# ssilverman16/particle_col_image_segmentation

Measured on AMD Instinct MI355X. Metric: Mpixels/sec segmented (5-ch 1024x1024 TIFF), ROI mask IoU=1.0, higher is better.
Workload: dtype f32 planes / u8 class maps / int32 labels / f64 ROI sums; 1 GPU; BASELINE config 2: batch of 64 frames 1024x1024x5 float32 per GPU, full kernel chain, inputs resident in HBM; frames_per_gpu=64, height=1024, width=1024, planes=5, parallelism=frames x1, launch=one hipGraph replay per step, 4 in flight, tie_fallback_frames_last_step=0, reference_nan_frames_rank0=0

## Files before the change

include/pcseg.h:

```cpp
#ifndef PCSEG_H
#define PCSEG_H

#include <stddef.h>
#include <stdint.h>

#ifdef __cplusplus
extern "C" {
#endif

typedef void *pcseg_stream_t;

enum pcseg_status {
    PCSEG_OK = 0,
    PCSEG_ERR_ARG = -1,
    PCSEG_ERR_HIP = -2,
    PCSEG_ERR_WORKSPACE = -3,
    PCSEG_ERR_CAPACITY = -4
};

enum pcseg_region_col {
    PCSEG_R_AREA = 0, PCSEG_R_SUM_ROW = 1, PCSEG_R_SUM_COL = 2,
    PCSEG_R_MIN_ROW = 3, PCSEG_R_MIN_COL = 4, PCSEG_R_MAX_ROW1 = 5, PCSEG_R_MAX_COL1 = 6,
    PCSEG_R_FIRST = 7, PCSEG_R_NCOLS = 8
};
// ... 71 lines not shown
int pcseg_fill_holes(const uint8_t *mask, uint8_t *out, int B, int H, int W,
                     void *workspace, size_t workspace_bytes, pcseg_stream_t stream);

size_t pcseg_local_maxima_workspace_bytes(int B, int H, int W);
int pcseg_local_maxima_i32(const int32_t *img, uint8_t *is_max, int32_t *markers, int32_t *counts,
                           int B, int H, int W, void *workspace, size_t workspace_bytes, pcseg_stream_t stream);

enum pcseg_ws_poison { PCSEG_WS_POISON_BORDER = 8, PCSEG_WS_POISON_LABEL = 16, PCSEG_WS_POISON_LEVEL2 = 32 };
size_t pcseg_watershed_workspace_bytes(int B, int H, int W);
void pcseg_watershed_counters(int64_t *out, int reset);
int pcseg_watershed4_f32(const float *img, int64_t frame_stride, const int32_t *markers, const uint8_t *mask,
                         int32_t *out, int32_t *tie_flags, int B, int H, int W, int mode,
                         void *workspace, size_t workspace_bytes, pcseg_stream_t stream);

size_t pcseg_merge_groups_workspace_bytes(int B, int list_cap);
int pcseg_merge_groups(const int32_t *dilated_labels, int keys_are_roots, const int64_t *stats,
                       const int32_t *region_list, const int32_t *n_list, int32_t *group_of, int32_t *n_groups,
                       int B, int H, int W, int cap, int list_cap, void *workspace, size_t workspace_bytes,
                       pcseg_stream_t stream);
int pcseg_merge_groups_runs(const uint32_t *dilated_bits, const int32_t *run_parent, const int64_t *stats,
                            const int32_t *region_list, const int32_t *n_list, int32_t *group_of, int32_t *n_groups,
                            int B, int H, int W, int cap, int list_cap, void *workspace, size_t workspace_bytes,
                            pcseg_stream_t stream);

int pcseg_merge_groups_fused(const uint32_t *dilated_bits, const int32_t *run_parent, const int64_t *stats,
                             const int32_t *region_lists, const int32_t *n_lists, int slot, int n_slots,
                             int32_t *group_of, int32_t *n_groups, int64_t *group_stats, int B, int H, int W, int cap,
                             void *workspace, size_t workspace_bytes, pcseg_stream_t stream);

int pcseg_merge_groups_fused_multi(const uint32_t *dilated_bits, const int32_t *run_parent, const int64_t *stats,
                                   const int32_t *region_lists, const int32_t *n_lists, const int32_t *slots, int n_masks,
                                   int n_slots, int32_t *group_of, int32_t *n_groups, int64_t *group_stats, int B, int H,
                                   int W, int cap, void *workspace, size_t workspace_bytes, pcseg_stream_t stream);

int pcseg_group_reduce(const int64_t *stats, const int32_t *region_list, const int32_t *n_list,
                       const int32_t *group_of, const int32_t *n_groups, int64_t *group_stats,
                       int B, int H, int W, int cap, int list_cap, pcseg_stream_t stream);

int pcseg_classify_regions(const int64_t *stats, const uint8_t *cls_out, const int32_t *counts,
                           const uint8_t *class_slot, const uint8_t *class_particle,
                           const int32_t *min_cell, const int32_t *min_cluster, int n_slots,
                           uint8_t *kind, uint8_t *slot_of, int32_t *cells, int64_t *particle_area,
                           int64_t *type_stats, int32_t *region_list, int32_t *n_list, int32_t *nan_flag,
                           int B, int cap, pcseg_stream_t stream);

int pcseg_nearest_dist_f64(const double *a, int na, const double *b, int nb, double *out_a, pcseg_stream_t stream);

size_t pcseg_overlap_workspace_bytes(int B, int H, int W);
int pcseg_remove_overlapping(const uint8_t *dapi, const uint8_t *other, double threshold, uint8_t *out,
                             int B, int H, int W, void *workspace, size_t workspace_bytes,
                             pcseg_stream_t stream);

typedef struct pcseg_table_inputs {
    int32_t B, cap, C, n_ratios;
    const int64_t *frame_ids;
    const int32_t *counts; const int64_t *stats; const uint8_t *cls_out; const double *cc_sums;
    const uint8_t *kind; const uint8_t *slot_of; const int32_t *cells;
    const int64_t *particle_area; const int64_t *overlap_area; const int64_t *type_stats; const int32_t *tie_flags;
    const int32_t *region_list; const int32_t *n_list;
    const int32_t *group_of[5]; const int32_t *n_groups[5]; const int64_t *group_stats[5];
    const int32_t *n_markers; const int64_t *ws_stats; const double *ws_sums;
    int32_t ratio_num[8]; int32_t ratio_den[8][4];
    const int32_t *overflow; const int32_t *ws_overflow; const int32_t *nan_flag;
} pcseg_table_inputs;
size_t pcseg_table_workspace_bytes(int B, int cap);
int pcseg_table_layout(const pcseg_table_inputs *in, int64_t *totals, void *workspace, size_t workspace_bytes,
// ... 92 lines not shown
```

particle_col_image_segmentation_amd/_lib.py:

```python
import ctypes
import os
from ctypes import c_char_p, c_double, c_float, c_int, c_int64, c_size_t, c_uint64, c_void_p

_HERE = os.path.dirname(os.path.abspath(__file__))
LIB_PATH = os.path.join(_HERE, "libpcseg.so")
_lib = None


class PcsegError(RuntimeError):
    pass


_P = c_void_p
_I = c_int
SIGNATURES = {
    "pcseg_version": (c_int, []),
    "pcseg_last_error": (c_char_p, []),
    "pcseg_device_count": (c_int, []),
    "pcseg_timing_enable": (None, [c_int]),
    "pcseg_timing_report": (c_int, [c_char_p, c_size_t]),
    "pcseg_argmax_planes_f32": (c_int, [_P, _P, _I, _I, _I, _I, _P]),
    "pcseg_median5_u8": (c_int, [_P, _P, _I, _I, _I, _P]),
    "pcseg_classmap_label_workspace_bytes": (c_size_t, [_I, _I, _I]),
    "pcseg_classmap_label_f32": (c_int, [_P, _I, _P, _P, _P, _I, _I, _I, _P, c_size_t, _P]),
    "pcseg_ccl_workspace_bytes": (c_size_t, [_I, _I, _I]),
    "pcseg_ccl8_equal_u8": (c_int, [_P, _P, _P, _I, _I, _I, _P, c_size_t, _P]),
    "pcseg_ccl8_bool": (c_int, [_P, _P, _P, _I, _I, _I, _P, c_size_t, _P]),
    "pcseg_ccl4_bool": (c_int, [_P, _P, _P, _I, _I, _I, _P, c_size_t, _P]),
    "pcseg_compact_labels": (c_int, [_P, _P, _P, _I, _I, _I, _P, c_size_t, _P]),
    "pcseg_region_reduce": (c_int, [_P, _P, _P, _I, _I, _I, _I, _I, _P, _P, _P, _P, _P]),
    "pcseg_region_reduce_n": (c_int, [_P, _P, _P, _P, _I, _I, _I, _I, _I, _P, _P, _P, _P, _P]),
    "pcseg_region_reduce_sel": (c_int, [_P, _P, _P, ctypes.c_uint64, _P, _I, _I, _I, _I, _I, _P, _P, _P, _P, _P]),
    "pcseg_region_init": (c_int, [_P, _I, _I, _I, _I, _I, _P, _P, _P, _P]),
    "pcseg_region_sums2": (c_int, [_P, _P, ctypes.c_uint64, _I, _P, _P, _I, _P, _P, _P, _P, _I, _I, _I, _I, _P]),
    "pcseg_threshold_lt_f32": (c_int, [_P, c_float, _P, _I, _I, _I, _P]),
    "pcseg_edt_workspace_bytes": (c_size_t, [_I, _I, _I]),
    "pcseg_edt_sq_u8": (c_int, [_P, _P, _I, _I, _I, _I, _P, c_size_t, _P]),
    "pcseg_edt_sq_lt_f32": (c_int, [_P, c_int64, c_float, _P, _P, _I, _I, _I, _P, c_size_t, _P]),
    "pcseg_dilate_disk_u8": (c_int, [_P, c_uint64, _I, _P, _I, _I, _I, _P, c_size_t, _P]),
    "pcseg_fill_particle": (c_int, [_P, _P, _I, _I, _I, _I, _I, _P, _I, _I, _I, _P, c_size_t, _P]),
    "pcseg_fill_holes_workspace_bytes": (c_size_t, [_I, _I, _I]),
    "pcseg_fill_holes": (c_int, [_P, _P, _I, _I, _I, _P, c_size_t, _P]),
    "pcseg_local_maxima_workspace_bytes": (c_size_t, [_I, _I, _I]),
    "pcseg_local_maxima_i32": (c_int, [_P, _P, _P, _P, _I, _I, _I, _P, c_size_t, _P]),
    "pcseg_watershed_workspace_bytes": (c_size_t, [_I, _I, _I]),
    "pcseg_watershed_counters": (None, [_P, _I]),
    "pcseg_watershed4_f32": (c_int, [_P, c_int64, _P, _P, _P, _P, _I, _I, _I, _I, _P, c_size_t, _P]),
    "pcseg_merge_groups_workspace_bytes": (c_size_t, [_I, _I]),
    "pcseg_merge_groups": (c_int, [_P, _I, _P, _P, _P, _P, _P, _I, _I, _I, _I, _I, _P, c_size_t, _P]),
    "pcseg_dilate_ccl_workspace_bytes": (c_size_t, [_I, _I, _I]),
    "pcseg_dilate_ccl_roots_u8": (c_int, [_P, c_uint64, _I, _P, _I, _I, _I, _P, c_size_t, _P]),
    "pcseg_dilate_ccl_runs_workspace_bytes": (c_size_t, [_I, _I, _I]),
    "pcseg_dilate_ccl_runs_u8": (c_int, [_P, c_uint64, _I, _P, _P, _I, _I, _I, _P, c_size_t, _P]),
    "pcseg_merge_groups_runs": (c_int, [_P, _P, _P, _P, _P, _P, _P, _I, _I, _I, _I, _I, _P, c_size_t, _P]),
    "pcseg_dilate_ccl_runs_multi_u8": (c_int, [_P, _P, _I, _I, _P, _P, _I, _I, _I, _P, c_size_t, _P]),
    "pcseg_merge_groups_fused_multi": (c_int, [_P, _P, _P, _P, _P, _P, _I, _I, _P, _P, _P, _I, _I, _I, _I, _P, c_size_t, _P]),
    "pcseg_merge_groups_fused": (c_int, [_P, _P, _P, _P, _P, _I, _I, _P, _P, _P, _I, _I, _I, _I, _P, c_size_t, _P]),
    "pcseg_group_reduce": (c_int, [_P, _P, _P, _P, _P, _P, _I, _I, _I, _I, _I, _P]),
    "pcseg_classify_regions": (c_int, [_P, _P, _P, _P, _P, _P, _P, _I, _P, _P, _P, _P, _P, _P, _P, _P, _I, _I, _P]),
    "pcseg_nearest_dist_f64": (c_int, [_P, _I, _P, _I, _P, _P]),
    "pcseg_overlap_workspace_bytes": (c_size_t, [_I, _I, _I]),
    "pcseg_remove_overlapping": (c_int, [_P, _P, c_double, _P, _I, _I, _I, _P, c_size_t, _P]),
    "pcseg_table_workspace_bytes": (c_size_t, [_I, _I]),
    "pcseg_table_layout": (c_int, [_P, _P, _P, c_size_t, _P]),
    "pcseg_table_write": (c_int, [_P, _P, _P, _P, _P, _P, c_size_t, _P]),
    "pcseg_cell_distances": (c_int, [_P, c_int64, _I, _P, c_double, c_double, _P, _I, _P, c_size_t, _P]),
    "pcseg_neighbours_workspace_bytes": (c_size_t, [c_int64, _I, _I, _I]),
    "pcseg_point_neighbours": (c_int, [_P, _P, _P, _P, c_int64, _I, _I, c_double, _P, _I, _P, _P, _P, _P, c_size_t, _P]),
    "pcseg_neighbours_pack_cells": (c_int, [_P, _I, _P, _I, _P, c_size_t, _P, _P, _P, _P, _P]),
    "pcseg_label_parent_workspace_bytes": (c_size_t, [_I, _I, _I, _I]),
    "pcseg_label_parent": (c_int, [_P, _P, _P, _P, _P, _P, _P, _P, _P, _P, _P, _I, _I, _I, _I, _P, c_size_t, _P]),
    "pcseg_refined_workspace_bytes": (c_size_t, [_I, _I]),
    "pcseg_refined_layout": (c_int, [_P, _P, _P, c_size_t, _P]),
    "pcseg_refined_table_write": (c_int, [_P, _P, c_size_t, _P, _P, _P, _P, _P, _P, _P, _P, c_size_t, _P]),
    "pcseg_surface_workspace_bytes": (c_size_t, [_I, _I, _I]),
    "pcseg_surface_points": (c_int, [_P, c_uint64, _P, _P, _P, _P, _P, c_int64, _I, _I, _I, _P, c_size_t, _P]),
    "pcseg_surface_distances": (c_int, [_P, _P, _P, c_int64, _P, _P, _P, _I, _I, _I, c_double, _P, _I, _I, _P, _P, _P, _P, _P, _P,
                                        c_size_t, _P]),
    "pcseg_surface_thresholds": (c_int, [_P, _I, c_double, _P]),
    "pcseg_surface_shells_workspace_bytes": (c_size_t, [_I, _I, _I]),
    "pcseg_surface_shells": (c_int, [_P, _P, _P, _I, _I, _I, c_double, _P, _I, _P, _P, c_size_t, _P]),
    "pcseg_surface_pack_cells": (c_int, [_P, _I, _P, _I, _P, c_size_t, _P, _P, _P, _P, _P]),
    "pcseg_surface_pack_refined": (c_int, [_P, _I, _P, _P, c_int64, _I, _P, _P]),
    "pcseg_region_shape_workspace_bytes": (c_size_t, [_I, _I, _I]),
    "pcseg_region_shape": (c_int, [_P, _P, _P, _P, _I, _I, _I, _I, _P, c_size_t, _P]),
    "pcseg_shape_properties": (c_int, [_P, _P, _P, _P, _I, _I, _P]),
    "pcseg_region_hull_workspace_bytes": (c_size_t, [_I, _I, _I, _I]),
    "pcseg_region_hull": (c_int, [_P, _P, _P, _P, _P, _I, _I, _I, _I, _P, c_size_t, _P]),
    "pcseg_hull_properties": (c_int, [_P, _P, _P, _P, _I, _I, _P]),
    "pcseg_nearest_label_workspace_bytes": (c_size_t, [_I, _I, _I]),
    "pcseg_nearest_label_i32": (c_int, [_P, _P, _I, _P, _P, _P, _I, _I, _I, _P, c_size_t, _P]),
    "pcseg_territory_labels": (c_int, [_P, _P, c_int64, _P, c_int64, _P]),
    "pcseg_territory_reduce": (c_int, [_P, _P, _P, c_int64, _I, _P, _I, _I, _I, _P]),
    "pcseg_territory_pairs_workspace_bytes": (c_size_t, [_I, _I]),
    "pcseg_territory_pairs": (c_int, [_P, _P, c_int64, _I, _P, _P, _P, _I, _I, _I, _P, c_size_t, _P]),
    "pcseg_territory_pairs_write": (c_int, [_I, _P, _P, _I, _I, _P, _P, _P, _P, _I, _P, c_size_t, _P]),
    "pcseg_otsu_hist_f32":(c_int, [_P, _P, _P, _I, _I, _I, _P]),
    "pcseg_otsu_f32": (c_int, [_P, _P, _P, _P, _I, _I, _I, _P]),
    "pcseg_morph3x3": (c_int, [_P, _P, _I, _I, _I, _I, _P]),
}


class TableInputs(ctypes.Structure):
    _fields_ = [("B", ctypes.c_int32), ("cap", ctypes.c_int32), ("C", ctypes.c_int32), ("n_ratios", ctypes.c_int32),
                ("frame_ids", _P),
                ("counts", _P), ("stats", _P), ("cls_out", _P), ("cc_sums", _P),
                ("kind", _P), ("slot_of", _P), ("cells", _P),
                ("particle_area", _P), ("overlap_area", _P), ("type_stats", _P), ("tie_flags", _P),
                ("region_list", _P), ("n_list", _P),
                ("group_of", _P * 5), ("n_groups", _P * 5), ("group_stats", _P * 5),
                ("n_markers", _P), ("ws_stats", _P), ("ws_sums", _P),
                ("ratio_num", ctypes.c_int32 * 8), ("ratio_den", (ctypes.c_int32 * 4) * 8),
                ("overflow", _P), ("ws_overflow", _P), ("nan_flag", _P)]


class RefinedInputs(ctypes.Structure):
    _fields_ = [("B", ctypes.c_int32), ("cap", ctypes.c_int32), ("n_slots", ctypes.c_int32),
                ("frame_ids", _P),
                ("counts", _P), ("kind", _P), ("slot_of", _P), ("cells", _P),
                ("n_markers", _P), ("ws_stats", _P),
                ("parent", _P), ("parent_px", _P), ("n_overlap", _P), ("cls_r", _P),
                ("kind_r", _P), ("slot_r", _P), ("cells_r", _P), ("type_stats_r", _P),
                ("nan_flag_r", _P),
                ("parent_overflow", _P)]


def load():
    global _lib
    if _lib is not None:
        return _lib
    path = os.environ.get("PCSEG_LIB") or LIB_PATH
    if not os.path.exists(path):
        raise PcsegError(
            "libpcseg.so is not built (%s). Run `python -m particle_col_image_segmentation_amd.build` "
            "or __graft_entry__.build(); there is no CPU fallback." % path)
    lib = ctypes.CDLL(path)
    for name, (res, args) in SIGNATURES.items():
        fn = getattr(lib, name)
        fn.restype = res
        fn.argtypes = args
    _lib = lib
    return lib


def check(rc, what):
    if rc != 0:
        msg = load().pcseg_last_error()
        raise PcsegError("%s failed (%d): %s" % (what, rc, msg.decode() if msg else "?"))
```

particle_col_image_segmentation_amd/build.py:

```python
import os
import subprocess
import sys

HERE = os.path.dirname(os.path.abspath(__file__))
CSRC = os.path.join(HERE, "csrc")
SOURCES = ["stencil.hip", "ccl.hip", "reduce.hip", "edt.hip", "watershed.hip", "tables.hip", "frontend.hip", "neighbours.hip", "refined.hip", "surface.hip", "shape.hip", "hull.hip", "voronoi.hip"]
LIB = os.path.join(HERE, "libpcseg.so")


def _stale():
    if not os.path.exists(LIB):
        return True
    t = os.path.getmtime(LIB)
    deps = [os.path.join(CSRC, f) for f in SOURCES + ["common.h", "tile_ops.h", "table_common.h", "label_reduce.h"]]
    deps.append(os.path.join(HERE, "..", "include", "pcseg.h"))
    return any(os.path.getmtime(d) > t for d in deps)


def build(force=False, verbose=False, out_dir=None, extra_flags=None):
    lib_path = LIB if out_dir is None else os.path.join(out_dir, "libpcseg.so")
    if out_dir is None and not force and not _stale():
        return LIB
    hipcc = os.environ.get("HIPCC", "/opt/rocm/bin/hipcc")
    objs = []
    procs = []
    obj_dir = os.path.join(HERE, "build") if out_dir is None else os.path.join(out_dir, "build")
    os.makedirs(obj_dir, exist_ok=True)
    flags = (extra_flags if extra_flags is not None else os.environ.get("PCSEG_EXTRA_FLAGS", "")).split()
    for src in SOURCES:
        obj = os.path.join(obj_dir, src.replace(".hip", ".o"))
        cmd = [hipcc, "--offload-arch=gfx950", "-O3", "-fPIC", "-std=c++17"] + flags + [
            "-c", os.path.join(CSRC, src), "-o", obj]
        if verbose:
            print(" ".join(cmd), file=sys.stderr)
        procs.append((src, subprocess.Popen(cmd, stdout=subprocess.PIPE, stderr=subprocess.STDOUT)))
        objs.append(obj)
    for src, p in procs:
        out, _ = p.communicate()
        if p.returncode != 0:
            raise RuntimeError("hipcc failed on %s:\n%s" % (src, out.decode()))
    cmd = [hipcc, "--offload-arch=gfx950", "-shared", "-fPIC", "-o", lib_path] + objs
    subprocess.check_call(cmd)
    return lib_path


if __name__ == "__main__":
    print(build(force="--force" in sys.argv, verbose=True))
# ... 1 lines not shown
```

particle_col_image_segmentation_amd/csrc/ccl.hip:

```cpp
#include <type_traits>

#include "common.h"
#include "tile_ops.h"

namespace pcseg {

constexpr int SCAN_PIX = 1024;

struct KeyEqU8 {
    const uint8_t *p;
    int W;
    int64_t n;
    __device__ __forceinline__ int operator()(int b, int r, int c) const { return p[b * n + rowoff(r, W) + c]; }
};
struct KeyNzU8 {
    const uint8_t *p;
    int W;
    int64_t n;
    __device__ __forceinline__ int operator()(int b, int r, int c) const { return p[b * n + rowoff(r, W) + c] != 0; }
};
struct KeyZeroU8 {
    const uint8_t *p;
    int W;
    int64_t n;
// ... 487 lines not shown
    }
    plan->parent = ws.parent;
    plan->blockcount = ws.blockcount;
    plan->nblk = ws.nblk;
    plan->corrupt = ws.corrupt;
    return PCSEG_OK;
}

int ccl_equal_u8_finish(const uint8_t *in, const CclPlan &plan, bool tile_pass_done, int *labels, int *counts, int B, int H, int W,
                        hipStream_t s)
{
    const KeyEqU8 keyfn{in, W, (int64_t)H * W};
    PCSEG_CHECK_HIP(hipMemsetAsync(plan.corrupt, 0, sizeof(int) * (size_t)B, s));
    dim3 tgrid((W + CCL_TW - 1) / CCL_TW, (H + CCL_TH - 1) / CCL_TH, B);
    if (!tile_pass_done) {
        PCSEG_LAUNCH((ccl_tile_kernel<KeyEqU8, true>), tgrid, dim3(256), 0, s, keyfn, plan.parent, H, W);
        PCSEG_CHECK_LAUNCH();
    }
    if (tgrid.x > 1 || tgrid.y > 1) {
        const int64_t border_px = (int64_t)((H - 1) / CCL_TH) * W + (int64_t)2 * ((W - 1) / CCL_TW) * H;
        dim3 bgrid((unsigned)((border_px + 255) / 256), B);
        PCSEG_LAUNCH((ccl_border_kernel<KeyEqU8, true>), bgrid, dim3(256), 0, s, keyfn, plan.parent, H, W, plan.corrupt);
        PCSEG_CHECK_LAUNCH();
    }
    return ccl_compact(plan.parent, plan.blockcount, plan.nblk, labels, counts, PredAll(), true, B, H, W, s, plan.corrupt);
}

__global__ void __launch_bounds__(256) roots_to_parent_kernel(const int *__restrict__ roots, int *__restrict__ parent, int64_t total)
{
    int64_t i = (int64_t)blockIdx.x * blockDim.x + threadIdx.x;
    if (i < total) parent[i] = roots[i] - 1;
}

struct MaskSet {
    unsigned long long bits[4];
    int n;
};
template <bool VEC>
__global__ void __launch_bounds__(256) set_bits_kernel(const uint8_t *__restrict__ in, MaskSet masks, unsigned *__restrict__ bits,
                                                        int H, int W, int nch, int B)
{
    constexpr int COLS = VEC ? 4 : 1;
    const int c = (blockIdx.x * 256 + threadIdx.x) * COLS;
    const int ch = blockIdx.y, b = blockIdx.z;
    if (c >= W) return;
    const uint8_t *src = in + (int64_t)b * H * W + c;
    unsigned w[4][COLS];
#pragma unroll
    for (int m = 0; m < 4; ++m)
#pragma unroll
        for (int j = 0; j < COLS; ++j) w[m][j] = 0;
#pragma unroll 1
    for (int j0 = 0; j0 < 32; j0 += 8) {
        unsigned v8[8];
#pragma unroll
        for (int j = 0; j < 8; ++j) {
            const uint8_t *at = src + rowoff(min(ch * 32 + j0 + j, H - 1), W);
            v8[j] = VEC ? *reinterpret_cast<const unsigned *>(at) : (unsigned)*at;
        }
#pragma unroll
        for (int j = 0; j < 8; ++j) {
#pragma unroll
            for (int q = 0; q < COLS; ++q) {
                const unsigned a = (v8[j] >> (8 * q)) & 255u;
                const unsigned long long sel = a < 64 ? (1ull << a) : 0ull;
#pragma unroll
                for (int m = 0; m < 4; ++m)
                    if (m < masks.n && (masks.bits[m] & sel)) w[m][q] |= 1u << (j0 + j);
            }
        }
// ... 741 lines not shown
```

particle_col_image_segmentation_amd/csrc/common.h:

```cpp
#pragma once
#include <hip/hip_runtime.h>
#include <stdint.h>
#include <stdio.h>
#include <string.h>

#include "../../include/pcseg.h"

namespace pcseg {

constexpr int WAVE = 64;

void set_error(const char *fmt, ...);

#define PCSEG_CHECK_HIP(expr)                                                              \
    do {                                                                                   \
        hipError_t _e = (expr);                                                            \
        if (_e != hipSuccess) {                                                            \
            pcseg::set_error("%s failed: %s (%s:%d)", #expr, hipGetErrorString(_e), __FILE__, __LINE__); \
            return PCSEG_ERR_HIP;                                                          \
        }                                                                                  \
    } while (0)

#define PCSEG_CHECK_LAUNCH()                                                               \
    do {                                                                                   \
        hipError_t _e = hipGetLastError();                                                 \
        if (_e != hipSuccess) {                                                            \
            pcseg::set_error("kernel launch failed: %s (%s:%d)", hipGetErrorString(_e), __FILE__, __LINE__); \
            return PCSEG_ERR_HIP;                                                          \
        }                                                                                  \
    } while (0)

#define PCSEG_REQUIRE(cond, msg)                                                           \
    do {                                                                                   \
        if (!(cond)) {                                                                     \
            pcseg::set_error("%s: %s", __func__, msg);                                     \
            return PCSEG_ERR_ARG;                                                          \
        }                                                                                  \
    } while (0)

// ... 222 lines not shown
            a = ga;
        }
        if (pb != b) {
            if (gb != pb) __hip_atomic_store(par + b, gb, __ATOMIC_RELAXED, __HIP_MEMORY_SCOPE_AGENT);
            b = gb;
        }
    }
    walk_corrupt(corrupt);
    return false;
}
__device__ __forceinline__ void unite_glb(int *par, int a, int b, int *corrupt = nullptr)
{
    for (;;) {
        if (!find2_glb(par, a, b, corrupt)) return;
        if (a == b) return;
        if (a < b) { int t = a; a = b; b = t; }
        int old = atomicMin(par + a, b);
        if (old == a) return;
        if (!walk_ok(a, old)) { walk_corrupt(corrupt); return; }
        a = old;
    }
}

struct CclPlan {
    int *parent;
    int *blockcount;
    int nblk;
    int *corrupt;
};
int ccl_plan(void *workspace, size_t workspace_bytes, int B, int H, int W, CclPlan *plan, const char *who);
int ccl_equal_u8_finish(const uint8_t *in, const CclPlan &plan, bool tile_pass_done, int *labels, int *counts, int B, int H, int W,
                        hipStream_t s);

}
```

particle_col_image_segmentation_amd/csrc/reduce.hip:

```cpp
#include "label_reduce.h"

namespace pcseg {

constexpr int RED_MAXC = 8;
constexpr int RED_ROWS = 16;

__device__ __forceinline__ void atomic_min_i64(long long *p, long long v) { atomicMin(p, v); }
__device__ __forceinline__ void atomic_max_i64(long long *p, long long v) { atomicMax(p, v); }

__global__ void __launch_bounds__(256) region_init_kernel(long long *__restrict__ stats, double *__restrict__ sums,
                                                           const int *__restrict__ counts, int cap, int C, int H, int W)
{
    const int b = blockIdx.y;
    const int idx = blockIdx.x * blockDim.x + threadIdx.x;
    const int l = idx >> 3, f = idx & 7;
    int nl = counts ? min(counts[b], cap) : cap;
    if (l >= nl) return;
    stats[((int64_t)b * cap + l) * 8 + f] = f == 3 ? (long long)H : (f == 4 ? (long long)W : (f == 7 ? 0x7FFFFFFFFFFFFFFFLL : 0LL));
    if (sums && f < C) sums[((int64_t)b * cap + l) * C + f] = 0.0;
}

__global__ void __launch_bounds__(256) region_reduce_kernel(const int *__restrict__ labels, const float *__restrict__ planes,
                                                             const uint8_t *__restrict__ cls, unsigned long long sel, int C, int H,
                                                             int W, int cap, long long *__restrict__ stats,
// ... 554 lines not shown
}

constexpr int MG_THREADS = 1024, MG_LDS = 4096;

struct LabelKeys {
    const int *lab;
    __device__ __forceinline__ int key(int fb, long long y, long long x, int H, int W) const
    {
        return lab[(int64_t)fb * H * W + y * W + x];
    }
};
struct RootKeys {
    const int *parent;
    __device__ __forceinline__ int key(int fb, long long y, long long x, int H, int W) const
    {
        const int *par = parent + (int64_t)fb * H * W;
        int k = par[y * W + x];
        if (k >= 0) k = (unsigned)k < (unsigned)(H * W) ? walk_root(par, k) : -1;
        return k + 1;
    }
};
struct RunRoots {
    const unsigned *bits;
    const int *parent;
    __device__ __forceinline__ int key(int fb, long long y, long long x, int H, int W) const
    {
        const int nch = (H + 31) / 32;
        const unsigned word = bits[((int64_t)fb * nch + (int)(y >> 5)) * W + x];
        const int j = (int)(y & 31);
        if (!((word >> j) & 1u)) return 0;
        const unsigned below = ~word & ((1u << j) - 1u);
        const int start = below ? 32 - __clz(below) : 0;
        return walk_root(parent + (int64_t)fb * H * W, (int)((y - j + start) * W + x)) + 1;
    }
};

template <typename Source>
__device__ __forceinline__ int centroid_key(const Source &src, const long long *st, int r, int fb, int H, int W, int cap)
{
    if (r < 0 || r >= cap) return 0;
    const long long a = st[(int64_t)r * 8 + 0];
    if (a <= 0) return 0;
    const long long y = st[(int64_t)r * 8 + 1] / a, x = st[(int64_t)r * 8 + 2] / a;
    if (y < 0 || y >= H || x < 0 || x >= W) return 0;
    return src.key(fb, y, x, H, W);
}

__device__ __forceinline__ void group_row_clear(long long *t, int H, int W)
{
    t[0] = 0; t[1] = 0; t[2] = 0; t[3] = H; t[4] = W; t[5] = 0; t[6] = 0; t[7] = 0;
}
__device__ __forceinline__ void group_row_add(long long *t, const long long *s, int f)
{
    if (f < 3) atomicAdd((unsigned long long *)&t[f], (unsigned long long)s[f]);
    else if (f < 5) atomicMin(&t[f], s[f]);
    else if (f < 7) atomicMax(&t[f], s[f]);
    else atomicAdd((unsigned long long *)&t[f], 1ull);
}

struct GroupTables {
    int *key, *gid, *first;
};

template <int THREADS, bool SUMS>
__device__ __forceinline__ int group_by_key(const GroupTables &t, int R, int *gof, int *wsum, const int *lst, const long long *st,
                                            long long *gs, int H, int W)
// ... 390 lines not shown
                                                 group_of, n_groups, nullptr, B, H, W, cap, list_cap, workspace, workspace_bytes, stream);
}

int pcseg_merge_groups_runs(const uint32_t *dilated_bits, const int32_t *run_parent, const int64_t *stats,
                            const int32_t *region_list, const int32_t *n_list, int32_t *group_of, int32_t *n_groups, int B, int H,
                            int W, int cap, int list_cap, void *workspace, size_t workspace_bytes, pcseg_stream_t stream)
{
    PCSEG_REQUIRE(dilated_bits && run_parent && stats && region_list && n_list && group_of && n_groups && workspace && cap >= 1 &&
                      list_cap >= 1 && check_shape(B, H, W),
                  "bad arguments");
    return merge_groups_launch<RunRoots, false>("merge_groups_runs", RunRoots{dilated_bits, run_parent}, stats, region_list, n_list,
                                                MergeSlots{}, 1, 1, group_of, n_groups, nullptr, B, H, W, cap, list_cap, workspace,
                                                workspace_bytes, stream);
}

int pcseg_merge_groups_fused_multi(const uint32_t *dilated_bits, const int32_t *run_parent, const int64_t *stats,
                                   const int32_t *region_lists, const int32_t *n_lists, const int32_t *slots, int n_masks, int n_slots,
                                   int32_t *group_of, int32_t *n_groups, int64_t *group_stats, int B, int H, int W, int cap,
                                   void *workspace, size_t workspace_bytes, pcseg_stream_t stream)
{
    PCSEG_REQUIRE(dilated_bits && run_parent && stats && region_lists && n_lists && slots && group_of && n_groups && group_stats &&
                      workspace && cap >= 1 && n_slots >= 1 && n_masks >= 1 && n_masks <= 4 && check_shape(B, H, W),
                  "bad arguments (1..4 masks)");
    MergeSlots ms;
    for (int m = 0; m < 4; ++m) {
        ms.slot[m] = m < n_masks ? slots[m] : 0;
        PCSEG_REQUIRE(ms.slot[m] >= 0 && ms.slot[m] < n_slots, "list slot out of range");
    }
    return merge_groups_launch<RunRoots, true>("merge_groups_fused", RunRoots{dilated_bits, run_parent}, stats, region_lists, n_lists, ms,
                                               n_masks, n_slots, group_of, n_groups, group_stats, B, H, W, cap, cap, workspace,
                                               workspace_bytes, stream);
}

int pcseg_merge_groups_fused(const uint32_t *dilated_bits, const int32_t *run_parent, const int64_t *stats,
                             const int32_t *region_lists, const int32_t *n_lists, int slot, int n_slots, int32_t *group_of,
                             int32_t *n_groups, int64_t *group_stats, int B, int H, int W, int cap, void *workspace,
                             size_t workspace_bytes, pcseg_stream_t stream)
{
    const int32_t slots[1] = {slot};
    return pcseg_merge_groups_fused_multi(dilated_bits, run_parent, stats, region_lists, n_lists, slots, 1, n_slots, group_of, n_groups,
                                          group_stats, B, H, W, cap, workspace, workspace_bytes, stream);
}

int pcseg_classify_regions(const int64_t *stats, const uint8_t *cls_out, const int32_t *counts, const uint8_t *class_slot,
                           const uint8_t *class_particle, const int32_t *min_cell, const int32_t *min_cluster, int n_slots,
                           uint8_t *kind, uint8_t *slot_of, int32_t *cells, int64_t *particle_area, int64_t *type_stats,
                           int32_t *region_list, int32_t *n_list, int32_t *nan_flag, int B, int cap, pcseg_stream_t stream)
{
    PCSEG_REQUIRE(stats && cls_out && counts && class_slot && class_particle && min_cell && min_cluster && kind && slot_of &&
                      cells && particle_area && type_stats && region_list && n_list && nan_flag && B >= 1 && cap >= 1 &&
                      n_slots >= 0 && n_slots <= CLS_T,
                  "bad arguments (class tables are HOST arrays: slot[256], particle[256], min_cell[n], min_cluster[n])");
    ClassTables tab;
    memcpy(tab.slot, class_slot, 256);
    memcpy(tab.particle, class_particle, 256);
    for (int t = 0; t < CLS_T; ++t) {
        tab.min_cell[t] = t < n_slots ? min_cell[t] : 0x7FFFFFFF;
        tab.min_cluster[t] = t < n_slots ? min_cluster[t] : 0x7FFFFFFF;
    }
    tab.n_slots = n_slots;
    PCSEG_LAUNCH(classify_regions_kernel, dim3(B), dim3(CLS_THREADS), 0, (hipStream_t)stream, (const long long *)stats, cls_out,
                       counts, tab, kind, slot_of, cells, (long long *)particle_area, (long long *)type_stats, region_list, n_list,
                       nan_flag, cap);
    PCSEG_CHECK_LAUNCH();
    return PCSEG_OK;
}
// ... 23 lines not shown
```

particle_col_image_segmentation_amd/ops.py:

```python
import collections
import ctypes
import functools

import torch

from . import _lib


def _stream():
    return ctypes.c_void_p(torch.cuda.current_stream().cuda_stream)


def _ptr(t):
    return ctypes.c_void_p(t.data_ptr()) if t is not None else ctypes.c_void_p(0)


def _req(t, dtype, ndim):
    if not isinstance(t, torch.Tensor) or not t.is_cuda:
        raise TypeError("expected a CUDA tensor (the HIP path has no CPU fallback)")
    if t.dtype == torch.bool and dtype == torch.uint8:
        t = t.view(torch.uint8)
    if t.dtype != dtype:
        raise TypeError("expected dtype %s, got %s" % (dtype, t.dtype))
    if t.dim() != ndim:
# ... 392 lines not shown
    bits = torch.empty((M, B, (H + 31) // 32, W), dtype=torch.int32, device=x.device)
    run_parent = torch.empty((M, B, H, W), dtype=torch.int32, device=x.device)
    nbytes = lib.pcseg_dilate_ccl_runs_workspace_bytes(B * M, H, W)
    ws = _ws(nbytes, x.device)
    vb = np.array([int(v) for v in value_bits_list], np.uint64)
    _lib.check(lib.pcseg_dilate_ccl_runs_multi_u8(_ptr(x), ctypes.c_void_p(vb.ctypes.data), M, int(radius), _ptr(bits), _ptr(run_parent),
                                                  B, H, W, _ptr(ws), nbytes, _stream()), "dilated_runs_multi")
    return bits, run_parent


def merge_groups_fused_multi(bits, run_parent, stats, region_lists, n_lists, slots):
    import numpy as np
    bits = _req(bits, torch.int32, 4)
    run_parent = _req(run_parent, torch.int32, 4)
    stats = _req(stats, torch.int64, 3)
    region_lists = _req(region_lists, torch.int32, 3)
    n_lists = _req(n_lists, torch.int32, 2)
    M, B, H, W = run_parent.shape
    cap = stats.shape[1]
    n_slots = region_lists.shape[1]
    if len(slots) != M or bits.shape[0] != M or region_lists.shape[2] != cap or tuple(n_lists.shape) != (B, n_slots):
        raise ValueError("masks / lists / region table do not match")
    dev = stats.device
    lib = _lib.load()
    group_of = torch.empty((M, B, cap), dtype=torch.int32, device=dev)
    n_groups = torch.empty((M, B), dtype=torch.int32, device=dev)
    gstats = torch.empty((M, B, cap, 8), dtype=torch.int64, device=dev)
    nbytes = lib.pcseg_merge_groups_workspace_bytes(B * M, cap)
    ws = _ws(nbytes, dev)
    sl = np.array([int(v) for v in slots], np.int32)
    _lib.check(lib.pcseg_merge_groups_fused_multi(_ptr(bits), _ptr(run_parent), _ptr(stats), _ptr(region_lists), _ptr(n_lists),
                                                  ctypes.c_void_p(sl.ctypes.data), M, n_slots, _ptr(group_of), _ptr(n_groups),
                                                  _ptr(gstats), B, H, W, cap, _ptr(ws), nbytes, _stream()), "merge_groups_fused_multi")
    return group_of, n_groups, gstats


def merge_groups_fused(bits, run_parent, stats, region_lists, n_lists, slot):
    bits = _req(bits, torch.int32, 3)
    run_parent = _req(run_parent, torch.int32, 3)
    stats = _req(stats, torch.int64, 3)
    region_lists = _req(region_lists, torch.int32, 3)
    n_lists = _req(n_lists, torch.int32, 2)
    B, H, W = run_parent.shape
    cap = stats.shape[1]
    n_slots = region_lists.shape[1]
    if region_lists.shape[2] != cap or tuple(n_lists.shape) != (B, n_slots):
        raise ValueError("region lists of shape %s / %s do not match the region table" % (tuple(region_lists.shape), tuple(n_lists.shape)))
    dev = stats.device
    lib = _lib.load()
    group_of = torch.empty((B, cap), dtype=torch.int32, device=dev)
    n_groups = torch.empty((B,), dtype=torch.int32, device=dev)
    gstats = torch.empty((B, cap, 8), dtype=torch.int64, device=dev)
    nbytes = lib.pcseg_merge_groups_workspace_bytes(B, cap)
    ws = _ws(nbytes, dev)
    _lib.check(lib.pcseg_merge_groups_fused(_ptr(bits), _ptr(run_parent), _ptr(stats), _ptr(region_lists), _ptr(n_lists), int(slot),
                                            n_slots, _ptr(group_of), _ptr(n_groups), _ptr(gstats), B, H, W, cap, _ptr(ws), nbytes,
                                            _stream()), "merge_groups_fused")
    return group_of, n_groups, gstats


def merge_groups(dilated_labels, stats, region_list, n_list, roots=False):
    dl = _req(dilated_labels, torch.int32, 3)
    stats = _req(stats, torch.int64, 3)
    region_list = _req(region_list, torch.int32, 2)
    n_list = _req(n_list, torch.int32, 1)
    B, H, W = dl.shape
# ... 724 lines not shown
```

particle_col_image_segmentation_amd/pipeline.py:

```python
import collections

import numpy as np
import torch

from . import ops
from . import tiff_analysis as ta
from .synth import BOUNDARY_PLANE, CELL_TYPES_5

RATIOS_7 = (("C13act", 1, (1, 0)), ("N15act", 3, (2, 3)), ("O17act", 5, (6, 5, 4)), ("O18act", 6, (6, 5, 4)))
RATIOS_5 = (("C13act", 1, (1, 0)), ("N15act", 3, (2, 3)))


class BatchResult(dict):

    _pending = None
    _slot = None
    _gen = 0

    def _check_alive(self):
        if self._slot is not None and self._slot.gen != self._gen:
            raise RuntimeError("this graph-mode result has been overwritten: its lane has replayed a later batch "
                               "(results stay valid until `lanes` further batches have been handed to run())")

    def done_events(self):
# ... 353 lines not shown
            ev = torch.cuda.Event()
            ev.record(st)
            done.append(ev)
        return dict(out), done

    def _class_stage(self, stack, res, denoised_ready=None):
        B, C, H, W = stack.shape
        cap = self.cap or max(1024, (H * W) // 64)
        tb = self.tables_
        z, labels, counts = ops.classmap_label(stack)
        res["denoised"] = z
        if denoised_ready is not None:
            denoised_ready.record(torch.cuda.current_stream())
        stats, cls_out, cc_sums, overflow = ops.region_reduce(labels, counts, cls=z, cap=cap, zero_sums=C)
        res.update(labels=labels, counts=counts, stats=stats, cls_out=cls_out, cc_sums=cc_sums, overflow=overflow)
        res.update(ops.classify_regions(stats, cls_out, counts, tb))
        res["groups"] = {}

    def _merge_all(self, stack, res):
        slots = self._merge_slots()
        if not slots:
            return
        B, C, H, W = stack.shape
        tb = self.tables_
        masks = []
        for s in slots:
            bits = 0
            for v in ([tb.slot_value[s]] if s < 4 else tb.slot_value):
                bits |= 1 << v
            masks.append(bits)
        keep = [k for k, m in enumerate(masks) if m]
        if not keep:
            return
        for lo in range(0, len(keep), 4):
            part = keep[lo:lo + 4]
            dbits, run_par = ops.dilated_runs_multi(res["denoised"], [masks[k] for k in part], ta.CELL_CLUSTER_DISTANCE_THRESHOLD // 2)
            gof, ng, gst = ops.merge_groups_fused_multi(dbits, run_par, res["stats"], res["region_list"], res["n_list"], [slots[k] for k in part])
            for m, k in enumerate(part):
                res["groups"][slots[k]] = {"group_of": gof[m], "n_groups": ng[m], "group_stats": gst[m]}

    def _fill_stage(self, stack, res):
        B = stack.shape[0]
        tb = self.tables_
        ds = res["denoised"]
        overlap = torch.zeros((B,), dtype=torch.int64, device=stack.device)
        if tb.particle_value is not None:
            for v in tb.cell_values:
                ds, overlap = ops.fill_particle(ds, tb.particle_value, v, tb.particle_value, ta.DILATION_RADIUS,
                                                ta.DISTANCE_THRESHOLD, overlap)
        res["recreated"] = ds
        res["overlap_area"] = overlap

    def _refine_chain(self, stack, res):
        B, C, H, W = stack.shape
        cap = self.cap or max(1024, (H * W) // 64)
        bm = stack[:, self.boundary_plane]
        d2, mask = ops.edt_sq_lt(bm, self.threshold)
        _, markers, n_markers = ops.local_maxima(d2, want_mask=False)
        ws_labels, tie_flags = ops.watershed(bm, markers, mask, mode=self.watershed_mode)
        res.update(mask=mask, markers=markers, n_markers=n_markers, ws_labels=ws_labels, tie_flags=tie_flags)
        ws_stats, _, ws_sums, ws_overflow = ops.region_reduce(ws_labels, n_markers, cap=cap, zero_sums=C)
        res.update(ws_stats=ws_stats, ws_sums=ws_sums, ws_overflow=ws_overflow)

    def _sums_stage(self, stack, res):
        cell_bits = 0
        for v in self.tables_.cell_values:
            cell_bits |= 1 << int(v)
        B, C, H, W = stack.shape
        aligned = all(t.data_ptr() % 16 == 0 for t in (res["labels"], res["ws_labels"], stack)) and res["denoised"].data_ptr() % 4 == 0
        if W % 4 == 0 and aligned:
# ... 179 lines not shown
```

Baseline: 17110 Mpixels/s.

## Merge regions directly via window union-find instead of dilated-run CCL

Replaces the dilate-then-CCL-on-runs path for cluster grouping with a direct region-level merge. The disk is convolved with itself to form a reach window, pairs of existing labels within that window are united in a small per-mask parent array, and a shared-memory hash deduplicates pairs. Group keys are then resolved per pixel by searching the disk neighbourhood. This avoids materialising dilated bitmaps and running pixel-level CCL over them, at the cost of a heavier per-pixel key lookup and global atomics for the unions.

```diff
diff --git a/include/pcseg.h b/include/pcseg.h
--- a/include/pcseg.h
+++ b/include/pcseg.h
@@ -127,6 +127,13 @@
                                    const int32_t *region_lists, const int32_t *n_lists, const int32_t *slots, int n_masks,
                                    int n_slots, int32_t *group_of, int32_t *n_groups, int64_t *group_stats, int B, int H,
                                    int W, int cap, void *workspace, size_t workspace_bytes, pcseg_stream_t stream);
+
+size_t pcseg_merge_regions_workspace_bytes(int B, int n_masks, int cap, int radius);
+int pcseg_merge_regions_multi(const uint8_t *cls, const int32_t *labels, const int32_t *counts, const uint64_t *value_bits,
+                              int n_masks, int radius, const int64_t *stats, const int32_t *region_lists,
+                              const int32_t *n_lists, const int32_t *slots, int n_slots, int32_t *group_of,
+                              int32_t *n_groups, int64_t *group_stats, int B, int H, int W, int cap, void *workspace,
+                              size_t workspace_bytes, pcseg_stream_t stream);
 
 int pcseg_group_reduce(const int64_t *stats, const int32_t *region_list, const int32_t *n_list,
                        const int32_t *group_of, const int32_t *n_groups, int64_t *group_stats,
diff --git a/particle_col_image_segmentation_amd/_lib.py b/particle_col_image_segmentation_amd/_lib.py
--- a/particle_col_image_segmentation_amd/_lib.py
+++ b/particle_col_image_segmentation_amd/_lib.py
@@ -55,6 +55,8 @@
     "pcseg_merge_groups_runs": (c_int, [_P, _P, _P, _P, _P, _P, _P, _I, _I, _I, _I, _I, _P, c_size_t, _P]),
     "pcseg_dilate_ccl_runs_multi_u8": (c_int, [_P, _P, _I, _I, _P, _P, _I, _I, _I, _P, c_size_t, _P]),
     "pcseg_merge_groups_fused_multi": (c_int, [_P, _P, _P, _P, _P, _P, _I, _I, _P, _P, _P, _I, _I, _I, _I, _P, c_size_t, _P]),
+    "pcseg_merge_regions_workspace_bytes": (c_size_t, [_I, _I, _I, _I]),
+    "pcseg_merge_regions_multi": (c_int, [_P, _P, _P, _P, _I, _I, _P, _P, _P, _P, _I, _P, _P, _P, _I, _I, _I, _I, _P, c_size_t, _P]),
     "pcseg_merge_groups_fused": (c_int, [_P, _P, _P, _P, _P, _I, _I, _P, _P, _P, _I, _I, _I, _I, _P, c_size_t, _P]),
     "pcseg_group_reduce": (c_int, [_P, _P, _P, _P, _P, _P, _I, _I, _I, _I, _I, _P]),
     "pcseg_classify_regions": (c_int, [_P, _P, _P, _P, _P, _P, _P, _I, _P, _P, _P, _P, _P, _P, _P, _P, _I, _I, _P]),
@@ -101,6 +103,9 @@
 }
 
 
+NEWER = {"pcseg_merge_regions_workspace_bytes", "pcseg_merge_regions_multi"}
+
+
 class TableInputs(ctypes.Structure):
     _fields_ = [("B", ctypes.c_int32), ("cap", ctypes.c_int32), ("C", ctypes.c_int32), ("n_ratios", ctypes.c_int32),
                 ("frame_ids", _P),
@@ -136,6 +141,8 @@
             "or __graft_entry__.build(); there is no CPU fallback." % path)
     lib = ctypes.CDLL(path)
     for name, (res, args) in SIGNATURES.items():
+        if name in NEWER and path != LIB_PATH and not hasattr(lib, name):
+            continue
         fn = getattr(lib, name)
         fn.restype = res
         fn.argtypes = args
diff --git a/particle_col_image_segmentation_amd/build.py b/particle_col_image_segmentation_amd/build.py
--- a/particle_col_image_segmentation_amd/build.py
+++ b/particle_col_image_segmentation_amd/build.py
@@ -4,7 +4,7 @@
 
 HERE = os.path.dirname(os.path.abspath(__file__))
 CSRC = os.path.join(HERE, "csrc")
-SOURCES = ["stencil.hip", "ccl.hip", "reduce.hip", "edt.hip", "watershed.hip", "tables.hip", "frontend.hip", "neighbours.hip", "refined.hip", "surface.hip", "shape.hip", "hull.hip", "voronoi.hip"]
+SOURCES = ["stencil.hip", "ccl.hip", "merge_regions.hip", "reduce.hip", "edt.hip", "watershed.hip", "tables.hip", "frontend.hip", "neighbours.hip", "refined.hip", "surface.hip", "shape.hip", "hull.hip", "voronoi.hip"]
 LIB = os.path.join(HERE, "libpcseg.so")
 
 
@@ -12,7 +12,7 @@
     if not os.path.exists(LIB):
         return True
     t = os.path.getmtime(LIB)
-    deps = [os.path.join(CSRC, f) for f in SOURCES + ["common.h", "tile_ops.h", "table_common.h", "label_reduce.h"]]
+    deps = [os.path.join(CSRC, f) for f in SOURCES + ["common.h", "tile_ops.h", "table_common.h", "label_reduce.h", "merge_window.h"]]
     deps.append(os.path.join(HERE, "..", "include", "pcseg.h"))
     return any(os.path.getmtime(d) > t for d in deps)
 
diff --git a/particle_col_image_segmentation_amd/csrc/ccl.hip b/particle_col_image_segmentation_amd/csrc/ccl.hip
--- a/particle_col_image_segmentation_amd/csrc/ccl.hip
+++ b/particle_col_image_segmentation_amd/csrc/ccl.hip
@@ -543,10 +543,6 @@
     if (i < total) parent[i] = roots[i] - 1;
 }
 
-struct MaskSet {
-    unsigned long long bits[4];
-    int n;
-};
 template <bool VEC>
 __global__ void __launch_bounds__(256) set_bits_kernel(const uint8_t *__restrict__ in, MaskSet masks, unsigned *__restrict__ bits,
                                                         int H, int W, int nch, int B)
diff --git a/particle_col_image_segmentation_amd/csrc/common.h b/particle_col_image_segmentation_amd/csrc/common.h
--- a/particle_col_image_segmentation_amd/csrc/common.h
+++ b/particle_col_image_segmentation_amd/csrc/common.h
@@ -5,6 +5,7 @@
 #include <string.h>
 
 #include "../../include/pcseg.h"
+#include "merge_window.h"
 
 namespace pcseg {
 
@@ -293,4 +294,12 @@
 int ccl_equal_u8_finish(const uint8_t *in, const CclPlan &plan, bool tile_pass_done, int *labels, int *counts, int B, int H, int W,
                         hipStream_t s);
 
-}
+struct MaskSet {
+    unsigned long long bits[4];
+    int n;
+};
+
+int merge_regions_front(const uint8_t *cls, const int *labels, const int *counts, const MaskSet &masks, const MergeWindow &win,
+                        int *parent, int B, int H, int W, int cap, hipStream_t s);
+
+}
diff --git a/particle_col_image_segmentation_amd/csrc/merge_regions.hip b/particle_col_image_segmentation_amd/csrc/merge_regions.hip
--- /dev/null
+++ b/particle_col_image_segmentation_amd/csrc/merge_regions.hip
@@ -0,0 +1,135 @@
+#include "common.h"
+
+namespace pcseg {
+
+constexpr int MR_TW = 64, MR_TH = 64, MR_ROWS = MR_TH + MW_MAX_REACH, MR_SEEN = 512, MR_BATCH = 4;
+
+__device__ __forceinline__ bool mask_has(unsigned long long bits, unsigned c) { return c < 64u && ((bits >> c) & 1ull); }
+
+__global__ void __launch_bounds__(256) merge_regions_init_kernel(int *__restrict__ parent, const int *__restrict__ counts, int B, int cap)
+{
+    const int b = blockIdx.y, m = blockIdx.z;
+    const int n = min(counts[b], cap);
+    const int i = blockIdx.x * 256 + threadIdx.x;
+    if (i < n) parent[((int64_t)m * B + b) * cap + i] = i;
+}
+
+__global__ void __launch_bounds__(256) merge_regions_front_kernel(const int *__restrict__ labels, const uint8_t *__restrict__ cls,
+                                                                   MaskSet masks, MergeWindow win, int *__restrict__ parent, int B,
+                                                                   int H, int W, int cap)
+{
+    __shared__ int lab[MR_ROWS][MR_TW + 1];
+    __shared__ unsigned long long inb[4][MR_ROWS], hd[4][MR_ROWS];
+    __shared__ unsigned long long seen[MR_SEEN];
+    __shared__ unsigned later[MW_MAX_REACH + 1];
+    const int reach = win.reach, own = MR_TW - 2 * reach;
+    const TileIndex ti = xcd_tile_index();
+    const int b = ti.z, r0 = ti.y * MR_TH, c0 = ti.x * own - reach;
+    const int lane = lane_id(), wv = threadIdx.x >> 6;
+    const int own_rows = min(MR_TH, H - r0), nrows = own_rows + reach;
+    const int col = c0 + lane;
+    const bool col_ok = col >= 0 && col < W;
+    const int cc = min(max(col, 0), W - 1);
+    const int64_t frame = (int64_t)b * H * W;
+    for (int i = threadIdx.x; i < MR_SEEN; i += 256) seen[i] = 0ull;
+    if (threadIdx.x <= MW_MAX_REACH) later[threadIdx.x] = win.later[threadIdx.x];
+
+    unsigned long long all_bits = 0ull;
+#pragma unroll
+    for (int m = 0; m < 4; ++m) all_bits |= m < masks.n ? masks.bits[m] : 0ull;
+    int any = 0;
+    for (int row0 = wv * MR_BATCH; row0 < nrows; row0 += 4 * MR_BATCH) {
+        unsigned cv[MR_BATCH];
+        int lv[MR_BATCH];
+#pragma unroll
+        for (int k = 0; k < MR_BATCH; ++k) cv[k] = cls[frame + rowoff(min(r0 + row0 + k, H - 1), W) + cc];
+#pragma unroll
+        for (int k = 0; k < MR_BATCH; ++k) {
+            const bool ok = col_ok && r0 + row0 + k < H && row0 + k < nrows;
+            if (!ok) cv[k] = 255u;
+            lv[k] = mask_has(all_bits, cv[k]) ? labels[frame + rowoff(min(r0 + row0 + k, H - 1), W) + cc] : 0;
+        }
+#pragma unroll
+        for (int k = 0; k < MR_BATCH; ++k) {
+            const int row = row0 + k;
+            if (row >= nrows) break;
+            const int left = __shfl_up(lv[k], 1);
+            const unsigned long long same = __ballot(lane > 0 && left == lv[k]);
+            lab[row][lane] = lv[k];
+#pragma unroll
+            for (int m = 0; m < 4; ++m) {
+                const unsigned long long in = m < masks.n ? __ballot(mask_has(masks.bits[m], cv[k])) : 0ull;
+                if (lane == 0) {
+                    inb[m][row] = in;
+                    hd[m][row] = in & ~((in << 1) & same);
+                }
+                any |= in != 0ull;
+            }
+        }
+    }
+    if (!__syncthreads_or(any)) return;
+
+    if (wv >= masks.n) return;
+    const int m = wv, row = lane;
+    if (row >= own_rows) return;
+    const unsigned long long own_cols = (~0ull >> (2 * reach)) << reach;
+    const unsigned long long in = inb[m][row];
+    if (!(in & own_cols)) return;
+    const unsigned long long head_lanes = hd[m][row] & own_cols, other_lanes = in & ~hd[m][row] & own_cols;
+    int *par = parent + ((int64_t)m * B + b) * cap;
+    int last_a = 0, last_b = 0;
+    auto pair = [&](int a, int o) {
+        if (a == o || (a == last_a && o == last_b)) return;
+        if ((unsigned)(a - 1) >= (unsigned)cap || (unsigned)(o - 1) >= (unsigned)cap) return;
+        last_a = a;
+        last_b = o;
+        const unsigned lo = (unsigned)min(a, o), hi = (unsigned)max(a, o);
+        const unsigned long long key = ((unsigned long long)(m + 1) << 60) | ((unsigned long long)hi << 30) | lo;
+        const unsigned slot = (unsigned)((hi * 2654435761u) ^ (lo * 40503u) ^ (unsigned)m) % MR_SEEN;
+        if (atomicExch(&seen[slot], key) != key) unite_glb(par, (int)hi - 1, (int)lo - 1);
+    };
+    for (int dy = 0; dy <= reach; ++dy) {
+        const unsigned long long msk = inb[m][row + dy];
+        if (!msk) continue;
+        const unsigned long long heads = hd[m][row + dy];
+        const unsigned long long srow = later[dy];
+        unsigned long long ends = srow & ~(srow >> 1);
+        while (ends) {
+            const int k = __ffsll((long long)ends) - 1 - reach;
+            ends &= ends - 1ull;
+            unsigned long long at = (k >= 0 ? heads >> k : heads << -k) & other_lanes;
+            while (at) {
+                const int p = __ffsll((long long)at) - 1;
+                at &= at - 1ull;
+                pair(lab[row][p], lab[row + dy][p + k]);
+            }
+        }
+        unsigned long long hs = head_lanes;
+        while (hs) {
+            const int p = __ffsll((long long)hs) - 1;
+            hs &= hs - 1ull;
+            const unsigned long long x = msk & (srow << (p - reach));
+            unsigned long long cand = x & (heads | ~(x << 1));
+            const int my = lab[row][p];
+            while (cand) {
+                const int q = __ffsll((long long)cand) - 1;
+                cand &= cand - 1ull;
+                pair(my, lab[row + dy][q]);
+            }
+        }
+    }
+}
+
+int merge_regions_front(const uint8_t *cls, const int *labels, const int *counts, const MaskSet &masks, const MergeWindow &win,
+                        int *parent, int B, int H, int W, int cap, hipStream_t s)
+{
+    PCSEG_LAUNCH(merge_regions_init_kernel, dim3((cap + 255) / 256, B, masks.n), dim3(256), 0, s, parent, counts, B, cap);
+    PCSEG_CHECK_LAUNCH();
+    const int own = MR_TW - 2 * win.reach;
+    PCSEG_LAUNCH(merge_regions_front_kernel, dim3((W + own - 1) / own, (H + MR_TH - 1) / MR_TH, B), dim3(256), 0, s, labels, cls, masks,
+                 win, parent, B, H, W, cap);
+    PCSEG_CHECK_LAUNCH();
+    return PCSEG_OK;
+}
+
+}
diff --git a/particle_col_image_segmentation_amd/csrc/merge_window.h b/particle_col_image_segmentation_amd/csrc/merge_window.h
--- /dev/null
+++ b/particle_col_image_segmentation_amd/csrc/merge_window.h
@@ -0,0 +1,46 @@
+#pragma once
+#include <stdint.h>
+
+namespace pcseg {
+
+constexpr int MW_MAX_RADIUS = 7;
+constexpr int MW_MAX_REACH = 2 * MW_MAX_RADIUS + 1;
+
+struct MergeWindow {
+    int radius;
+    int reach;
+    uint32_t disk[2 * MW_MAX_RADIUS + 1];
+    uint32_t later[MW_MAX_REACH + 1];
+};
+
+inline void mw_minkowski(const uint32_t *a, int ha, const uint32_t *b, int hb, uint32_t *c)
+{
+    const int na = 2 * ha + 1, nb = 2 * hb + 1;
+    for (int i = 0; i < na + nb - 1; ++i) c[i] = 0;
+    for (int i = 0; i < na; ++i)
+        for (int k = 0; k < na; ++k)
+            if ((a[i] >> k) & 1u)
+                for (int j = 0; j < nb; ++j) c[i + j] |= b[j] << k;
+}
+
+inline int merge_window_build(int radius, MergeWindow *w)
+{
+    if (radius < 0 || radius > MW_MAX_RADIUS) return -1;
+    const int r = radius, reach = 2 * r + 1;
+    w->radius = r;
+    w->reach = reach;
+    for (int i = 0; i < 2 * MW_MAX_RADIUS + 1; ++i) w->disk[i] = 0;
+    for (int i = 0; i <= MW_MAX_REACH; ++i) w->later[i] = 0;
+    for (int dy = -r; dy <= r; ++dy)
+        for (int dx = -r; dx <= r; ++dx)
+            if (dx * dx + dy * dy <= r * r) w->disk[dy + r] |= 1u << (dx + r);
+    uint32_t two[4 * MW_MAX_RADIUS + 1], s[2 * MW_MAX_REACH + 1];
+    const uint32_t n8[3] = {7u, 7u, 7u};
+    mw_minkowski(w->disk, r, w->disk, r, two);
+    mw_minkowski(two, 2 * r, n8, 1, s);
+    for (int dy = 0; dy <= reach; ++dy) w->later[dy] = s[dy + reach];
+    w->later[0] &= ~((2u << reach) - 1u);
+    return 0;
+}
+
+}
diff --git a/particle_col_image_segmentation_amd/csrc/reduce.hip b/particle_col_image_segmentation_amd/csrc/reduce.hip
--- a/particle_col_image_segmentation_amd/csrc/reduce.hip
+++ b/particle_col_image_segmentation_amd/csrc/reduce.hip
@@ -610,6 +610,39 @@
         const unsigned below = ~word & ((1u << j) - 1u);
         const int start = below ? 32 - __clz(below) : 0;
         return walk_root(parent + (int64_t)fb * H * W, (int)((y - j + start) * W + x)) + 1;
+    }
+};
+
+struct RegionRoots {
+    const int *labels;
+    const uint8_t *cls;
+    const int *parent;
+    MaskSet masks;
+    unsigned disk[2 * MW_MAX_RADIUS + 1];
+    int radius, B, cap;
+    __device__ __forceinline__ int key(int fb, long long y, long long x, int H, int W) const
+    {
+        const int m = fb / B, b = fb - m * B;
+        const int64_t frame = (int64_t)b * H * W;
+        const int *par = parent + (int64_t)fb * cap;
+        const unsigned long long bits = masks.bits[m];
+        auto root_at = [&](long long yy, long long xx) -> int {
+            const unsigned c = cls[frame + yy * W + xx];
+            if (c >= 64u || !((bits >> c) & 1ull)) return 0;
+            const int l = labels[frame + yy * W + xx];
+            return (l >= 1 && l <= cap) ? walk_root(par, l - 1) + 1 : 0;
+        };
+        int k = root_at(y, x);
+        for (int dy = -radius; dy <= radius && k == 0; ++dy) {
+            const long long yy = y + dy;
+            if (yy < 0 || yy >= H) continue;
+            const unsigned row = disk[dy + radius];
+            for (int dx = -radius; dx <= radius && k == 0; ++dx) {
+                const long long xx = x + dx;
+                if (((row >> (dx + radius)) & 1u) && xx >= 0 && xx < W) k = root_at(yy, xx);
+            }
+        }
+        return k;
     }
 };
 
@@ -1066,6 +1099,61 @@
                                                workspace_bytes, stream);
 }
 
+static GroupTables merge_regions_carve(Carver &cv, size_t BM, int cap, int **parent)
+{
+    *parent = cv.take<int>(BM * cap);
+    return merge_groups_carve(cv, BM, cap);
+}
+
+size_t pcseg_merge_regions_workspace_bytes(int B, int n_masks, int cap, int radius)
+{
+    if (B < 1 || n_masks < 1 || n_masks > 4 || cap < 1 || radius < 0 || radius > MW_MAX_RADIUS) return 0;
+    Carver cv(nullptr, 0);
+    int *parent;
+    merge_regions_carve(cv, (size_t)B * n_masks, cap, &parent);
+    return cv.off;
+}
+
+int pcseg_merge_regions_multi(const uint8_t *cls, const int32_t *labels, const int32_t *counts, const uint64_t *value_bits,
+                              int n_masks, int radius, const int64_t *stats, const int32_t *region_lists, const int32_t *n_lists,
+                              const int32_t *slots, int n_slots, int32_t *group_of, int32_t *n_groups, int64_t *group_stats, int B,
+                              int H, int W, int cap, void *workspace, size_t workspace_bytes, pcseg_stream_t stream)
+{
+    PCSEG_REQUIRE(cls && labels && counts && value_bits && stats && region_lists && n_lists && slots && group_of && n_groups &&
+                      group_stats && workspace && cap >= 1 && n_slots >= 1 && n_masks >= 1 && n_masks <= 4 && check_shape(B, H, W),
+                  "bad arguments (1..4 masks)");
+    MergeWindow win;
+    PCSEG_REQUIRE(merge_window_build(radius, &win) == 0, "no window table for this radius (0..7): use the run path");
+    MergeSlots ms;
+    RegionRoots src;
+    src.masks.n = n_masks;
+    for (int m = 0; m < 4; ++m) {
+        ms.slot[m] = m < n_masks ? slots[m] : 0;
+        PCSEG_REQUIRE(ms.slot[m] >= 0 && ms.slot[m] < n_slots, "list slot out of range");
+        src.masks.bits[m] = m < n_masks ? (unsigned long long)value_bits[m] : 0ull;
+    }
+    Carver cv(workspace, workspace_bytes);
+    int *parent;
+    merge_regions_carve(cv, (size_t)B * n_masks, cap, &parent);
+    if (!cv.ok()) {
+        set_error("merge_regions: workspace too small (%zu < %zu)", workspace_bytes, cv.off);
+        return PCSEG_ERR_WORKSPACE;
+    }
+    const int rc = merge_regions_front(cls, labels, counts, src.masks, win, parent, B, H, W, cap, (hipStream_t)stream);
+    if (rc) return rc;
+    src.labels = labels;
+    src.cls = cls;
+    src.parent = parent;
+    for (int i = 0; i < 2 * MW_MAX_RADIUS + 1; ++i) src.disk[i] = win.disk[i];
+    src.radius = radius;
+    src.B = B;
+    src.cap = cap;
+    const size_t used = align_up((size_t)B * n_masks * cap * sizeof(int));
+    return merge_groups_launch<RegionRoots, true>("merge_regions", src, stats, region_lists, n_lists, ms, n_masks, n_slots, group_of,
+                                                  n_groups, group_stats, B, H, W, cap, cap, (char *)workspace + used,
+                                                  workspace_bytes - used, stream);
+}
+
 int pcseg_merge_groups_fused(const uint32_t *dilated_bits, const int32_t *run_parent, const int64_t *stats,
                              const int32_t *region_lists, const int32_t *n_lists, int slot, int n_slots, int32_t *group_of,
                              int32_t *n_groups, int64_t *group_stats, int B, int H, int W, int cap, void *workspace,
diff --git a/particle_col_image_segmentation_amd/ops.py b/particle_col_image_segmentation_amd/ops.py
--- a/particle_col_image_segmentation_amd/ops.py
+++ b/particle_col_image_segmentation_amd/ops.py
@@ -448,6 +448,42 @@
     _lib.check(lib.pcseg_merge_groups_fused_multi(_ptr(bits), _ptr(run_parent), _ptr(stats), _ptr(region_lists), _ptr(n_lists),
                                                   ctypes.c_void_p(sl.ctypes.data), M, n_slots, _ptr(group_of), _ptr(n_groups),
                                                   _ptr(gstats), B, H, W, cap, _ptr(ws), nbytes, _stream()), "merge_groups_fused_multi")
+    return group_of, n_groups, gstats
+
+
+def merge_regions_supported(radius):
+    lib = _lib.load()
+    return hasattr(lib, "pcseg_merge_regions_multi") and lib.pcseg_merge_regions_workspace_bytes(1, 1, 1, int(radius)) > 0
+
+
+def merge_regions_multi(x, labels, counts, value_bits_list, radius, stats, region_lists, n_lists, slots):
+    import numpy as np
+    x = _req(x, torch.uint8, 3)
+    labels = _req(labels, torch.int32, 3)
+    counts = _req(counts, torch.int32, 1)
+    stats = _req(stats, torch.int64, 3)
+    region_lists = _req(region_lists, torch.int32, 3)
+    n_lists = _req(n_lists, torch.int32, 2)
+    B, H, W = x.shape
+    M = len(value_bits_list)
+    cap = stats.shape[1]
+    n_slots = region_lists.shape[1]
+    if (len(slots) != M or tuple(labels.shape) != (B, H, W) or counts.shape[0] != B or stats.shape[0] != B
+            or region_lists.shape[0] != B or region_lists.shape[2] != cap or tuple(n_lists.shape) != (B, n_slots)):
+        raise ValueError("masks / labels / lists / region table do not match")
+    dev = stats.device
+    lib = _lib.load()
+    group_of = torch.empty((M, B, cap), dtype=torch.int32, device=dev)
+    n_groups = torch.empty((M, B), dtype=torch.int32, device=dev)
+    gstats = torch.empty((M, B, cap, 8), dtype=torch.int64, device=dev)
+    nbytes = lib.pcseg_merge_regions_workspace_bytes(B, M, cap, int(radius))
+    ws = _ws(nbytes, dev)
+    vb = np.array([int(v) for v in value_bits_list], np.uint64)
+    sl = np.array([int(v) for v in slots], np.int32)
+    _lib.check(lib.pcseg_merge_regions_multi(_ptr(x), _ptr(labels), _ptr(counts), ctypes.c_void_p(vb.ctypes.data), M, int(radius),
+                                             _ptr(stats), _ptr(region_lists), _ptr(n_lists), ctypes.c_void_p(sl.ctypes.data), n_slots,
+                                             _ptr(group_of), _ptr(n_groups), _ptr(gstats), B, H, W, cap, _ptr(ws), nbytes, _stream()),
+               "merge_regions_multi")
     return group_of, n_groups, gstats
 
 
diff --git a/particle_col_image_segmentation_amd/pipeline.py b/particle_col_image_segmentation_amd/pipeline.py
--- a/particle_col_image_segmentation_amd/pipeline.py
+++ b/particle_col_image_segmentation_amd/pipeline.py
@@ -409,10 +409,16 @@
         keep = [k for k, m in enumerate(masks) if m]
         if not keep:
             return
+        radius = ta.CELL_CLUSTER_DISTANCE_THRESHOLD // 2
+        by_regions = ops.merge_regions_supported(radius)
         for lo in range(0, len(keep), 4):
             part = keep[lo:lo + 4]
-            dbits, run_par = ops.dilated_runs_multi(res["denoised"], [masks[k] for k in part], ta.CELL_CLUSTER_DISTANCE_THRESHOLD // 2)
-            gof, ng, gst = ops.merge_groups_fused_multi(dbits, run_par, res["stats"], res["region_list"], res["n_list"], [slots[k] for k in part])
+            if by_regions:
+                gof, ng, gst = ops.merge_regions_multi(res["denoised"], res["labels"], res["counts"], [masks[k] for k in part], radius,
+                                                       res["stats"], res["region_list"], res["n_list"], [slots[k] for k in part])
+            else:
+                dbits, run_par = ops.dilated_runs_multi(res["denoised"], [masks[k] for k in part], radius)
+                gof, ng, gst = ops.merge_groups_fused_multi(dbits, run_par, res["stats"], res["region_list"], res["n_list"], [slots[k] for k in part])
             for m, k in enumerate(part):
                 res["groups"][slots[k]] = {"group_of": gof[m], "n_groups": ng[m], "group_stats": gst[m]}
 
```

Result: slower. 16700 Mpixels/s (-2.4%).
